# david-m-rosen/Optimization

Hardware: AMD Instinct MI355X
Metric: TNT Steihaug-CG HVP+inner-product throughput (higher is better)
Workload: dtype f64

## Files before the change

optimization_amd/csrc/context.hip:

```cpp
#include "mi_internal.h"
#include <chrono>
#include <cstring>
#include <strings.h>
#include <unistd.h>

#include <dlfcn.h>

namespace mi {

static thread_local char g_err[1024] = "";

void set_error(const char *fmt, ...) {
  va_list ap;
  va_start(ap, fmt);
  vsnprintf(g_err, sizeof(g_err), fmt, ap);
  va_end(ap);
}

int hip_fail(hipError_t e, const char *what, const char *file, int line) {
  set_error("HIP error %d (%s) in %s at %s:%d", (int)e, hipGetErrorString(e), what, file, line);
  (void)hipGetLastError();
  if (e == hipErrorNoDevice || e == hipErrorInvalidDevice) return MI_ERR_NO_DEVICE;
  if (e == hipErrorOutOfMemory) return MI_ERR_OOM;
  return MI_ERR_HIP;
// ... 171 lines not shown
using namespace mi;

namespace {
struct OptionDesc {
  const char *name;
  int (*set)(mi_ctx *, long);
  bool integer = false;
};
#define OPT_BOOL(FN, FIELD) \
  int FN(mi_ctx *c, long v) { c->FIELD = v != 0; return MI_OK; }
OPT_BOOL(opt_force_slot_path, force_slot_path)
OPT_BOOL(opt_force_lockstep, force_lockstep)
OPT_BOOL(opt_no_dirgram, no_dirgram)
OPT_BOOL(opt_dirgram_direct, dirgram_direct)
OPT_BOOL(opt_force_uniform_grid, cfg.force_uniform_grid)
OPT_BOOL(opt_no_fold, cfg.no_fold)
OPT_BOOL(opt_halo_push_late, cfg.halo_push_late)
OPT_BOOL(opt_no_packed, cfg.no_packed)
OPT_BOOL(opt_no_window, cfg.no_window)
OPT_BOOL(opt_no_win_bounds, cfg.no_win_bounds)
OPT_BOOL(opt_no_far_computed, cfg.no_far_computed)
OPT_BOOL(opt_words16, cfg.words16)
OPT_BOOL(opt_no_spmm_stream, cfg.no_spmm_stream)
OPT_BOOL(opt_no_spmm_win, cfg.no_spmm_win)
OPT_BOOL(opt_no_spmm_sweep, cfg.no_spmm_sweep)
OPT_BOOL(opt_no_zero_copy, cfg.no_zero_copy)
OPT_BOOL(opt_no_polled_sync, cfg.no_polled_sync)
OPT_BOOL(opt_no_update_mfma, cfg.no_update_mfma)
OPT_BOOL(opt_halo_rprime, cfg.halo_rprime)
OPT_BOOL(opt_no_gram_half, cfg.no_gram_half)
OPT_BOOL(opt_so3_no_quat, cfg.so3_no_quat)
OPT_BOOL(opt_so3_no_rquat, cfg.so3_no_rquat)
OPT_BOOL(opt_early_s, cfg.early_s)
OPT_BOOL(opt_no_update_pair, cfg.no_update_pair)
OPT_BOOL(opt_two_kernel_step, cfg.two_kernel_step)
OPT_BOOL(opt_warn_generic, warn_generic)
#undef OPT_BOOL
int opt_max_grid(mi_ctx *c, long v) {
  c->max_grid = (int)std::min<long>(kMaxGrid, std::max<long>(1, v));
  return MI_OK;
}
int opt_wide_quad(mi_ctx *c, long v) {
  c->cfg.wide_quad = v < 0 ? -1 : v != 0;
  return MI_OK;
}
int opt_wide_window(mi_ctx *c, long v) {
  c->cfg.wide_window = v < 0 ? -1 : v != 0;
  return MI_OK;
}
int opt_so3_sort_nbr(mi_ctx *c, long v) {
  c->cfg.so3_sort_nbr = (int)v;
  return MI_OK;
}
int opt_sweep_zsegs(mi_ctx *c, long v) {
  c->cfg.sweep_zsegs = (int)std::max<long>(0, std::min<long>(v, 1024));
  return MI_OK;
}
int opt_reanchor(mi_ctx *c, long v) {
  c->cfg.reanchor = (int)std::max<long>(0, std::min<long>(v, 1 << 20));
  return MI_OK;
}
int opt_ipc_timeout_ms(mi_ctx *c, long v) {
  c->cfg.ipc_timeout_ms = std::max<long>(0, v);
  return MI_OK;
}
const OptionDesc kOptions[] = {
    {"FORCE_SLOT_PATH", opt_force_slot_path}, {"FORCE_LOCKSTEP", opt_force_lockstep},
    {"NO_DIRGRAM", opt_no_dirgram}, {"DIRGRAM_DIRECT", opt_dirgram_direct}, {"MAX_GRID", opt_max_grid, true},
    {"FORCE_UNIFORM_GRID", opt_force_uniform_grid}, {"IPC_TIMEOUT_MS", opt_ipc_timeout_ms, true},
    {"NO_FOLD", opt_no_fold}, {"HALO_PUSH_LATE", opt_halo_push_late}, {"NO_PACKED", opt_no_packed},
    {"NO_WINDOW", opt_no_window}, {"NO_WIN_BOUNDS", opt_no_win_bounds}, {"NO_FAR_COMPUTED", opt_no_far_computed},
    {"WORDS16", opt_words16}, {"NO_SPMM_STREAM", opt_no_spmm_stream}, {"NO_SPMM_WIN", opt_no_spmm_win},
    {"NO_SPMM_SWEEP", opt_no_spmm_sweep}, {"SWEEP_ZSEGS", opt_sweep_zsegs, true},
    {"NO_ZERO_COPY", opt_no_zero_copy}, {"NO_POLLED_SYNC", opt_no_polled_sync}, {"WIDE_QUAD", opt_wide_quad, true}, {"WIDE_WINDOW", opt_wide_window, true},
    {"NO_UPDATE_MFMA", opt_no_update_mfma}, {"HALO_RPRIME", opt_halo_rprime}, {"NO_GRAM_HALF", opt_no_gram_half}, {"SO3_NO_QUAT", opt_so3_no_quat}, {"SO3_NO_RQUAT", opt_so3_no_rquat}, {"EARLY_S", opt_early_s}, {"NO_UPDATE_PAIR", opt_no_update_pair}, {"TWO_KERNEL_STEP", opt_two_kernel_step}, {"SO3_SORT_NBR", opt_so3_sort_nbr, true},
    {"WARN_GENERIC", opt_warn_generic}, {"REANCHOR", opt_reanchor, true},
};
bool option_value(const OptionDesc &o, const char *e, long *v) {
  char *end = nullptr;
  *v = strtol(e, &end, 0);
  if (end != e && *end == '\0') return true;
  if (o.integer) {
    fprintf(stderr, "[mi355opt] warning: MI355OPT_%s=\"%s\" is not an integer; ignored (the default stays)\n", o.name, e);
    return false;
  }
  *v = (!strcasecmp(e, "no") || !strcasecmp(e, "false") || !strcasecmp(e, "off")) ? 0 : 1;
  return true;
}
void config_from_env(mi_ctx *ctx) {
  for (const OptionDesc &o : kOptions) {
    char name[64];
    snprintf(name, sizeof(name), "MI355OPT_%s", o.name);
    long v = 0;
    if (const char *e = getenv(name))
      if (option_value(o, e, &v)) (void)o.set(ctx, v);
  }
  static bool warned = false;
  if (warned || !environ) return;
  warned = true;
  for (char **ep = environ; *ep; ++ep) {
    if (strncmp(*ep, "MI355OPT_", 9) != 0) continue;
    const char *nm = *ep + 9, *eq = strchr(nm, '=');
    const size_t len = eq ? (size_t)(eq - nm) : strlen(nm);
    bool known = false;
    for (const OptionDesc &o : kOptions) known |= strlen(o.name) == len && strncmp(o.name, nm, len) == 0;
    for (const char *h : {"LIB", "COMM", "BUILD_TAG", "EXTRA_CFLAGS", "NO_UNITY"})
      known |= strlen(h) == len && strncmp(h, nm, len) == 0;
    known |= len >= 6 && strncmp(nm, "BENCH_", 6) == 0;
// ... 297 lines not shown
```

optimization_amd/csrc/mi_internal.h:

```cpp
#pragma once

#include <hip/hip_runtime.h>

#include <cstdarg>
#include <cstdint>
#include <cstdio>
#include <cstring>
#include <map>
#include <string>
#include <set>
#include <vector>

#include "mi355opt.h"

namespace mi {

constexpr int kWave = 64;
constexpr int kBlock = 1024;
constexpr int kWaves = kBlock / kWave;
constexpr int kMaxP = 8;
constexpr int kMaxGrid = 512;
constexpr int kMaxRows = 1024;
constexpr int kMaxComps = 64;
constexpr int kNumXCD = 8;
// ... 41 lines not shown
};
static_assert(sizeof(CgState) <= 128, "the CG state is meant to fit one 128-byte line");
struct CgConst {
  double Delta, Delta_2, epsilon;
  unsigned long long max_iterations;
  unsigned long long rag0, rag_per;
};
enum CgMode { CG_RUN = 0, CG_KERNEL_PENDING = 1, CG_APPLY_SIGMA = 2, CG_DONE = 3 };

struct Config {
  bool force_uniform_grid = false;
  long ipc_timeout_ms = 0;
  bool no_fold = false;
  bool halo_push_late = false;
  bool no_packed = false;
  bool no_window = false;
  bool no_win_bounds = false;
  bool no_far_computed = false;
  bool words16 = false;
  bool no_spmm_stream = false;
  bool no_spmm_sweep = true;
  int sweep_zsegs = 0;
  bool no_spmm_win = false;
  bool no_zero_copy = false;
  int wide_quad = -1;
  int wide_window = -1;
  bool no_polled_sync = false;
  bool two_kernel_step = false;
  int reanchor = 25;
  bool no_update_pair = false;
  bool no_gram_half = false;
  bool no_update_mfma = false;
  bool halo_rprime = false;
  bool early_s = false;
  bool so3_no_rquat = false;
  bool so3_no_quat = false;
  int so3_sort_nbr = 0;
};

struct KTimer {
  bool enabled = false;
  std::vector<std::pair<hipEvent_t, hipEvent_t>> pending;
  size_t launches = 0;
  double total_ms = 0;
};

}

struct mi_ctx {
  int device = -1;
  hipStream_t stream = nullptr;
  char device_name[128] = {0};
  int num_cu = 256;
  bool uniform_grid = false;
  int max_grid = 512;
  std::multimap<size_t, void *> pool_free;
  std::map<void *, size_t> pool_all;
  size_t pool_bytes = 0;
  void *control_slab = nullptr;
  double *partials = nullptr;
  double *partials_b = nullptr;
  double *partials2 = nullptr;
  double *partials_user = nullptr;
  double *scalars = nullptr;
  double *host_scalars = nullptr;
  mi::CgState *cg = nullptr;
// ... 367 lines not shown
```

optimization_amd/csrc/stpcg.hip:

```cpp
#include "comm_ipc.h"
#include "mi_internal.h"
#include "stiefel_core.h"

#include <cmath>
#include <type_traits>

using namespace mi;

namespace {

enum { PRE_NONE = 0, PRE_DIAG = 1, PRE_BLOCK3 = 2, PRE_EXTERNAL = 3 };

__device__ __forceinline__ void publish(HostStatus *hs, unsigned long long launches, int done) {
  __hip_atomic_store(&hs->word, (uint64_t)(launches << 1) | (uint64_t)(done ? 1 : 0), __ATOMIC_RELAXED,
                     __HIP_MEMORY_SCOPE_SYSTEM);
}

#define CG_FIELDS(X)                                                                               \
  X(sk_M_pk) X(sk_M_2) X(pk_M_2) X(target_rk_norm) X(rv) X(alpha) X(beta)                          \
  X(kappa) X(sigma) X(skplus1_M_2) X(M_norm) X(k) X(launches) X(mode) X(exit_reason)
__device__ __forceinline__ CgState load_state(const CgState *__restrict__ src) {
  CgState s;
#define X(f) s.f = src->f;
  CG_FIELDS(X)
// ... 257 lines not shown
    s.mode = CG_DONE;
    s.exit_reason = MI_STPCG_EXIT_RESIDUAL;
    s.M_norm = sqrt(0.0);
  }
  store_state(st, s);
  publish(hs, 0, s.mode == CG_DONE);
}

struct DirGramArgs {
  const double *X, *Y, *S;
  double *gpartials;
  double *gdir;
  int ns;
};

#ifdef MI_FOLD_STAMPS
}
extern "C" __attribute__((visibility("default"))) int mi_debug_fold_stamp_buffer(void *dev_ptr) {
  return (int)hipMemcpyToSymbol(HIP_SYMBOL(mi::g_fold_stamps), &dev_ptr, sizeof(dev_ptr));
}
namespace {
#endif

template <int SP>
struct DirGramLds {
  static constexpr int value = (SymIdx<SP>::NS * kWaves > kWaves + 1) ? SymIdx<SP>::NS * kWaves : kWaves + 1;
};
template <>
struct DirGramLds<0> {
  static constexpr int value = kWaves + 1;
};
static_assert(kWaves + 1 >= kIpcVals, "LDS of the folded exchange");

#define CG_KERNEL_ATTR
#define CG_UPDATE_NAME k_cg_update
#define CG_PUPDATE_NAME k_cg_pupdate
#include "stpcg_kernels.inc"
#undef CG_KERNEL_ATTR
#undef CG_UPDATE_NAME
#undef CG_PUPDATE_NAME
#define CG_KERNEL_ATTR __attribute__((amdgpu_num_sgpr(80), amdgpu_waves_per_eu(8, 8)))
#define CG_UPDATE_NAME k_cg_update_s80
#define CG_PUPDATE_NAME k_cg_pupdate_s80
#include "stpcg_kernels.inc"
#undef CG_KERNEL_ATTR
#undef CG_UPDATE_NAME
#undef CG_PUPDATE_NAME

template <class F>
__device__ __forceinline__ void reduce_rows_1x512(const double *__restrict__ partials, int count, double &out, double *lds,
                                                  F &&after_issue) {
  const int lane = threadIdx.x & 63, w = threadIdx.x >> 6;
  double t[8];
#pragma unroll
  for (int j = 0; j < 8; ++j) t[j] = 0.0;
  if (w == 0) {
#pragma unroll
    for (int j = 0; j < 8; ++j) {
      const int r = lane + 64 * j;
      if (r < count) t[j] = partials[r];
    }
  }
  after_issue();
  if (w == 0) {
    double v = 0;
#pragma unroll
    for (int j = 0; j < 8; ++j) v += t[j];
    v = wave_reduce_sum(v);
    if (lane == 0) lds[0] = v;
  }
  __syncthreads();
  out = lds[0];
  __syncthreads();
}

__global__ __launch_bounds__(kBlock) __attribute__((amdgpu_waves_per_eu(8, 8))) void k_cg_pupdate_early(
    size_t n, CgConst cc, const CgState *__restrict__ st_in, CgState *__restrict__ st_out,
    const double *__restrict__ partials_b, int nparts_b, const double *__restrict__ v, double *__restrict__ p,
    double *__restrict__ s, HostStatus *hs, double *__restrict__ trace, size_t trace_cap, DirGramArgs dg) {
  __shared__ double lds[kWaves + 1];
// ... 224 lines not shown
__global__ __launch_bounds__(kBlock) void k_cg_dirgram2(size_t nrows, const CgState *__restrict__ st,
                                                        const double *__restrict__ va, const double *__restrict__ vb,
                                                        DirGramArgs dg) {
  static_assert(SP >= 1 && SP <= 4, "narrow rows");
  __shared__ double lds[SymIdx<SP>::NS * kWaves];
  if (st->mode != CG_RUN) return;
  double Sm[SP * SP], Ga[SP * SP], Gb[SP * SP];
#pragma unroll
  for (int i = 0; i < SP * SP; ++i) { Ga[i] = 0; Gb[i] = 0; Sm[i] = dg.S[i]; }
  const size_t stride = (size_t)gridDim.x * kBlock;
  for (size_t row = (size_t)blockIdx.x * kBlock + threadIdx.x; row < nrows; row += stride) {
    double x[SP], y[SP], a[SP], b[SP];
#pragma unroll
    for (int c = 0; c < SP; ++c) {
      x[c] = dg.X[row * SP + c]; y[c] = dg.Y[row * SP + c]; a[c] = va[row * SP + c]; b[c] = vb[row * SP + c];
    }
#pragma unroll
    for (int j = 0; j < SP; ++j) {
      double ta = 0, tb = 0;
#pragma unroll
      for (int i = 0; i < SP; ++i) { ta += a[i] * Sm[i * SP + j]; tb += b[i] * Sm[i * SP + j]; }
#pragma unroll
      for (int i = 0; i < SP; ++i) {
        Ga[i * SP + j] += y[i] * a[j] - x[i] * ta;
        Gb[i * SP + j] += y[i] * b[j] - x[i] * tb;
      }
    }
  }
  store_sym_partials<SP>(Ga, lds, dg.gpartials);
  __syncthreads();
  store_sym_partials<SP>(Gb, lds, dg.gpartials + (size_t)SymIdx<SP>::NS * kMaxRows);
}

template <int SP>
__global__ __launch_bounds__(StBlk<SP>::threads) void k_cg_init_dirgram(size_t nrows, const double *__restrict__ g,
                                                            double *__restrict__ r, double *__restrict__ p,
                                                            double *__restrict__ s, double *__restrict__ partials,
                                                            DirGramArgs dg) {
  constexpr int BLK = StBlk<SP>::threads, NW = StBlk<SP>::waves;
  constexpr bool WIDE = SP > 4;
  __shared__ double lds[SymIdx<SP>::NS * NW];
  __shared__ double SmL[WIDE ? SP * SP : 1];
  double Sm[WIDE ? 1 : SP * SP], G[SP * SP];
#pragma unroll
  for (int i = 0; i < SP * SP; ++i) G[i] = 0;
  if (WIDE) {
    if (threadIdx.x < SP * SP) SmL[threadIdx.x] = dg.S[threadIdx.x];
    __syncthreads();
  } else {
#pragma unroll
    for (int i = 0; i < SP * SP; ++i) Sm[WIDE ? 0 : i] = dg.S[i];
  }
  double acc[1] = {0};
  const size_t stride = (size_t)gridDim.x * BLK;
  for (size_t row = (size_t)blockIdx.x * BLK + threadIdx.x; row < nrows; row += stride) {
    double x[SP], y[SP], gv[SP], pv[SP];
#pragma unroll
    for (int c = 0; c < SP; ++c) { x[c] = dg.X[row * SP + c]; y[c] = dg.Y[row * SP + c]; gv[c] = g[row * SP + c]; }
#pragma unroll
    for (int c = 0; c < SP; ++c) {
      pv[c] = -gv[c];
      r[row * SP + c] = gv[c];
      s[row * SP + c] = 0 * gv[c];
      p[row * SP + c] = pv[c];
      acc[0] += gv[c] * gv[c];
    }
    if (WIDE) asm volatile("" ::: "memory");
#pragma unroll
    for (int b = 0; b < SP; ++b) {
      double t = 0;
#pragma unroll
      for (int a = 0; a < SP; ++a) t += pv[a] * (WIDE ? SmL[a * SP + b] : Sm[WIDE ? 0 : a * SP + b]);
#pragma unroll
      for (int a = 0; a < SP; ++a) G[a * SP + b] += y[a] * pv[b] - x[a] * t;
    }
  }
  store_sym_partials<SP>(G, lds, dg.gpartials);
  __syncthreads();
  block_partials_store_w<1, NW>(acc, lds, partials);
}

__global__ __launch_bounds__(kBlock) void k_cg_gdir_init(const double *__restrict__ partials, int count, int ns,
                                                         const double *__restrict__ slots, int from_slots,
                                                         double *__restrict__ gdir) {
  if (!from_slots) {
    gdir_from_rows(partials, count, ns, gdir);
    return;
  }
  if (threadIdx.x < ns) {
    const double v = slots[threadIdx.x];
    gdir[SLOT_GDIR_P + threadIdx.x] = v;
    gdir[threadIdx.x] = -v;
  }
}

__global__ __launch_bounds__(kBlock) void k_cg_gdir_anchor(const double *__restrict__ partials, int count, int ns,
// ... 179 lines not shown
  hipStream_t st = ctx->stream;
  const int grid = (pre == PRE_BLOCK3) ? grid_for(ctx, n / 3, 2) : grid_for(ctx, n, 4);
  {
    const size_t n2 = n >> 1, step = (size_t)grid * kBlock;
    cc.rag0 = (n2 / step) * step;
    cc.rag_per = (n2 - cc.rag0 + (size_t)grid - 1) / (size_t)grid;
  }
  const bool recur = dgp && pre == PRE_NONE && !ctx->dirgram_direct;
  const int gns = dgp ? dgp->p * (dgp->p + 1) / 2 : 0;
  const DirGramArgs dga = dgp ? DirGramArgs{dgp->X, dgp->Y, dgp->S, ctx->partials2,
                                            recur ? ctx->scalars + SLOT_GDIR : nullptr, gns}
                              : DirGramArgs{nullptr, nullptr, nullptr, nullptr, nullptr, 0};
  const int sp = (dgp && !recur) ? dgp->p : 0;
  const int kc = recur ? dir_comps(dgp->p) : 3;
  double *slots_g = ctx->scalars + SLOT_GRAM;
  double *slots_a = ctx->scalars + SLOT_CG, *slots_b = ctx->scalars + SLOT_CG + 4;
  CgState *st0 = ctx->cg, *st1 = ctx->cg1;
  const bool folded = sharded && recur && kc <= kIpcVals && comm_fold_enabled(ctx) && !ctx->force_slot_path;
  bool rprime = false;
  if (recur && !folded && dgp->halo_A) {
    const int st_rp = comm_rprime_prepare(ctx, dgp->halo_A, &rprime);
    if (st_rp != MI_OK) {
      mi_vec_destroy(r);
      mi_vec_destroy(p);
      mi_vec_destroy(Hp);
      if (v) mi_vec_destroy(v);
      return st_rp;
    }
  }
  const bool init_fused = recur && n == dgp->n * (size_t)dgp->p;
  const bool gdir_in_scalar_init = recur && !sharded && !rows;
  const bool twok = ctx->cfg.two_kernel_step && recur && dgp->twok && dgp->p == 3 && !sharded && !rows && !lockstep &&
                    init_fused && gdir_in_scalar_init;
  CgState *st_final = st0;
  double *tr = tcap ? ctx->trace_dev : nullptr;
  int ret = MI_OK;
  ctx->cg_live = st0;

#define CG_CHECK(expr)   \
  do {                   \
    int _s = (expr);     \
    if (_s != MI_OK) {   \
      ret = _s;          \
      goto cleanup;      \
    }                    \
  } while (0)
#define LAUNCH_PRE(KERNEL, ...)                                                                   \
  switch (pre) {                                                                                  \
    case PRE_NONE: hipLaunchKernelGGL((KERNEL<PRE_NONE>), dim3(grid), dim3(kBlock), 0, st, __VA_ARGS__); break;     \
    case PRE_DIAG: hipLaunchKernelGGL((KERNEL<PRE_DIAG>), dim3(grid), dim3(kBlock), 0, st, __VA_ARGS__); break;     \
    case PRE_BLOCK3: hipLaunchKernelGGL((KERNEL<PRE_BLOCK3>), dim3(grid), dim3(kBlock), 0, st, __VA_ARGS__); break; \
    default: hipLaunchKernelGGL((KERNEL<PRE_EXTERNAL>), dim3(grid), dim3(kBlock), 0, st, __VA_ARGS__); break;       \
  }
#define LAUNCH_UPDATE(FS)                                                                              \
  switch (pre) {                                                                                       \
    case PRE_NONE: hipLaunchKernelGGL((k_cg_update<PRE_NONE, FS>), dim3(grid), dim3(kBlock), 0, st, UPD_ARGS, NoFold{}); break;     \
    case PRE_DIAG: hipLaunchKernelGGL((k_cg_update<PRE_DIAG, FS>), dim3(grid), dim3(kBlock), 0, st, UPD_ARGS, NoFold{}); break;     \
    case PRE_BLOCK3: hipLaunchKernelGGL((k_cg_update<PRE_BLOCK3, FS>), dim3(grid), dim3(kBlock), 0, st, UPD_ARGS, NoFold{}); break; \
    default: hipLaunchKernelGGL((k_cg_update<PRE_EXTERNAL, FS>), dim3(grid), dim3(kBlock), 0, st, UPD_ARGS, NoFold{}); break;       \
  }

  if (init_fused) {
    KScope ks(ctx, MI_K_CG_INIT);
    const size_t nrows = dgp->n;
#define INIT_DG(SPV)                                                                                       \
  hipLaunchKernelGGL(k_cg_init_dirgram<SPV>, dim3(grid), dim3(StBlk<SPV>::threads), 0, st, nrows, (const double *)g->d, \
                     r->d, p->d, s_out->d, ctx->partials_b, dga)
    switch (dgp->p) {
      case 1: INIT_DG(1); break;
      case 2: INIT_DG(2); break;
      case 3: INIT_DG(3); break;
      case 4: INIT_DG(4); break;
      case 5: INIT_DG(5); break;
      case 6: INIT_DG(6); break;
      case 7: INIT_DG(7); break;
      default: INIT_DG(8); break;
    }
#undef INIT_DG
  } else {
    KScope ks(ctx, MI_K_CG_INIT);
    LAUNCH_PRE(k_cg_init, n, (const double *)g->d, pred, r->d, vd, p->d, s_out->d, ctx->partials_b);
  }
  if (pre == PRE_EXTERNAL) {
    if (P->apply_project) CG_CHECK(P->apply_project(P, r, v, prm->constraint_At));
    else CG_CHECK(P->apply(P, r, v));
    hipLaunchKernelGGL(k_cg_dot_rv<true>, dim3(grid), dim3(kBlock), 0, st, n, (const CgState *)st0,
                       (const double *)r->d, (const double *)v->d, p->d, ctx->partials_b);
  }
  if (dgp) {
    const size_t nrows = dgp->n;
    if (!init_fused) {
      switch (dgp->p) {
        case 1: hipLaunchKernelGGL(k_cg_dirgram<1>, dim3(grid), dim3(kBlock), 0, st, nrows, (const double *)p->d, dga); break;
        case 2: hipLaunchKernelGGL(k_cg_dirgram<2>, dim3(grid), dim3(kBlock), 0, st, nrows, (const double *)p->d, dga); break;
        case 3: hipLaunchKernelGGL(k_cg_dirgram<3>, dim3(grid), dim3(kBlock), 0, st, nrows, (const double *)p->d, dga); break;
        case 4: hipLaunchKernelGGL(k_cg_dirgram<4>, dim3(grid), dim3(kBlock), 0, st, nrows, (const double *)p->d, dga); break;
        case 5: hipLaunchKernelGGL(k_cg_dirgram<5>, dim3(grid), dim3(StBlk<5>::threads), 0, st, nrows, (const double *)p->d, dga); break;
        case 6: hipLaunchKernelGGL(k_cg_dirgram<6>, dim3(grid), dim3(StBlk<6>::threads), 0, st, nrows, (const double *)p->d, dga); break;
        case 7: hipLaunchKernelGGL(k_cg_dirgram<7>, dim3(grid), dim3(StBlk<7>::threads), 0, st, nrows, (const double *)p->d, dga); break;
        default: hipLaunchKernelGGL(k_cg_dirgram<8>, dim3(grid), dim3(StBlk<8>::threads), 0, st, nrows, (const double *)p->d, dga); break;
// ... 81 lines not shown
                             ctx->status_dev, tr, tcap, dga);
        }
        st_final = nxt;
        continue;
      }
      if (dgp) {
        CG_CHECK(H->apply_dir(H, p, Hp, recur ? -1 : grid, &nparts));
      } else if (H->apply_dots) {
        CG_CHECK(H->apply_dots(H, p, Hp, &nparts));
      } else {
        CG_CHECK(H->apply(H, p, Hp));
        CG_CHECK(launch_dot3_partials(ctx, n, p->d, Hp->d, &nparts));
      }
      ++hvp;
#define UPD_ARGS                                                                                      \
  n, cc, (const CgState *)st0, st1, (const double *)ctx->partials, nparts,                              \
      (const double *)(recur ? slots_g : slots_a), (const double *)p->d, (const double *)Hp->d, pred,  \
      s_out->d, r->d, vd, ctx->partials_b, dga
      if (recur) {
#define UPD_RECUR(KN, FS, FT, FV)                                                                                  \
  switch (kc) {                                                                                                    \
    case 4: hipLaunchKernelGGL((KN<PRE_NONE, FS, 4, FT>), dim3(grid), dim3(kBlock), 0, st, UPD_ARGS, FV); break;   \
    case 6: hipLaunchKernelGGL((KN<PRE_NONE, FS, 6, FT>), dim3(grid), dim3(kBlock), 0, st, UPD_ARGS, FV); break;   \
    case 9: hipLaunchKernelGGL((KN<PRE_NONE, FS, 9, FT>), dim3(grid), dim3(kBlock), 0, st, UPD_ARGS, FV); break;   \
    default: hipLaunchKernelGGL((k_cg_update_s80<PRE_NONE, FS, 16, FT>), dim3(grid), dim3(kBlock), 0, st, UPD_ARGS, FV); break; \
  }
#define UPD_WIDE(FS)                                                                                                        \
  switch (kc) {                                                                                                             \
    case 18: hipLaunchKernelGGL((k_cg_update<PRE_NONE, FS, 18, NoFold>), dim3(grid), dim3(kBlock), 0, st, UPD_ARGS, NoFold{}); break; \
    case 24: hipLaunchKernelGGL((k_cg_update<PRE_NONE, FS, 24, NoFold>), dim3(grid), dim3(kBlock), 0, st, UPD_ARGS, NoFold{}); break; \
    case 31: hipLaunchKernelGGL((k_cg_update<PRE_NONE, FS, 31, NoFold>), dim3(grid), dim3(kBlock), 0, st, UPD_ARGS, NoFold{}); break; \
    default: hipLaunchKernelGGL((k_cg_update<PRE_NONE, FS, 39, NoFold>), dim3(grid), dim3(kBlock), 0, st, UPD_ARGS, NoFold{}); break; \
  }
        if (kc > 16) {
          if (sharded) CG_CHECK(reduce_rows_allreduce(ctx, ctx->partials, nparts, kc, slots_g));
          else if (rows) CG_CHECK(comm_allreduce_rows(ctx, ctx->partials, kc));
          KScope ks(ctx, MI_K_CG_UPDATE);
          if (sharded) { UPD_WIDE(true); } else { UPD_WIDE(false); }
        } else if (sharded && folded) {
          const FoldArgs fold_a = comm_fold_next(ctx);
          KScope ks(ctx, MI_K_CG_UPDATE);
          UPD_RECUR(k_cg_update_s80, false, FoldArgs, fold_a);
        } else if (sharded) {
          CG_CHECK(reduce_rows_allreduce(ctx, ctx->partials, nparts, kc, slots_g));
          KScope ks(ctx, MI_K_CG_UPDATE);
          UPD_RECUR(k_cg_update_s80, true, NoFold, NoFold{});
        } else {
          if (rows) CG_CHECK(comm_allreduce_rows(ctx, ctx->partials, kc));
          KScope ks(ctx, MI_K_CG_UPDATE);
          UPD_RECUR(k_cg_update, false, NoFold, NoFold{});
        }
#undef UPD_RECUR
#undef UPD_WIDE
      } else if (sharded) {
        CG_CHECK(reduce_rows_allreduce(ctx, ctx->partials, nparts, 3, slots_a));
        KScope ks(ctx, MI_K_CG_UPDATE);
        LAUNCH_UPDATE(true);
      } else {
        if (rows) CG_CHECK(comm_allreduce_rows(ctx, ctx->partials, 3));
        KScope ks(ctx, MI_K_CG_UPDATE);
        LAUNCH_UPDATE(false);
      }
#undef UPD_ARGS
      if (pre == PRE_EXTERNAL) {
        if (P->apply_project) CG_CHECK(P->apply_project(P, r, v, prm->constraint_At));
        else CG_CHECK(P->apply(P, r, v));
        hipLaunchKernelGGL(k_cg_dot_rv<false>, dim3(grid), dim3(kBlock), 0, st, n, (const CgState *)st1,
                           (const double *)r->d, (const double *)v->d, p->d, ctx->partials_b);
      }
#define PUPD_ARGS                                                                                          \
  n, cc, (const CgState *)st1, st0, (const double *)ctx->partials_b, grid, (const double *)slots_b,        \
      (const double *)vd, p->d, s_out->d, ctx->status_dev, tr, tcap, dga
#define PUPD(KN, FS, SPV) \
  hipLaunchKernelGGL((KN<FS, SPV>), dim3(grid), dim3(kBlock), 0, st, PUPD_ARGS, NoFold{})
#define LAUNCH_PUPD(KN0, KN1, FS)               \
  switch (sp) {                                 \
    case 0: PUPD(KN0, FS, 0); break;            \
    case 1: PUPD(KN1, FS, 1); break;            \
    case 2: PUPD(k_cg_pupdate, FS, 2); break;   \
    case 3: PUPD(k_cg_pupdate, FS, 3); break;   \
    default: PUPD(k_cg_pupdate, FS, 4); break;  \
  }
      if (sharded && folded) {
        const FoldArgs fold_b = comm_fold_next(ctx);
        FoldPush fp{fold_b, HaloPush{}};
        const bool push = dgp && dgp->halo_A && k + 1 < prm->max_iterations &&
                          comm_halo_fold_next(ctx, dgp->halo_A, dgp->p, p->d, &fp.h);
        KScope ks(ctx, MI_K_CG_PUPDATE);
        if (push)
          hipLaunchKernelGGL((k_cg_pupdate_s80<false, 0, FoldPush>), dim3(grid), dim3(kBlock), 0, st, PUPD_ARGS, fp);
        else
          hipLaunchKernelGGL((k_cg_pupdate_s80<false, 0, FoldArgs>), dim3(grid), dim3(kBlock), 0, st, PUPD_ARGS, fold_b);
      } else if (sharded) {
        CG_CHECK(reduce_rows_allreduce(ctx, ctx->partials_b, grid, 1, slots_b));
        if (rprime) CG_CHECK(comm_rprime_exchange(ctx, dgp->halo_A, dgp->p, r->d, nullptr, 0));
        KScope ks(ctx, MI_K_CG_PUPDATE);
        LAUNCH_PUPD(k_cg_pupdate_s80, k_cg_pupdate_s80, true);
      } else {
        if (rows && rprime) CG_CHECK(comm_rprime_exchange(ctx, dgp->halo_A, dgp->p, r->d, ctx->partials_b, 1));
        else if (rows) CG_CHECK(comm_allreduce_rows(ctx, ctx->partials_b, 1));
        KScope ks(ctx, MI_K_CG_PUPDATE);
        const bool early = sp == 0 && !rows && ctx->cfg.early_s && grid <= 512 && cc.rag0 <= 2ull * (size_t)grid * kBlock &&
                           (n >> 1) < ((size_t)1 << 31);
        if (early)
          hipLaunchKernelGGL(k_cg_pupdate_early, dim3(grid), dim3(kBlock), 0, st, n, cc, (const CgState *)st1, st0,
                             (const double *)ctx->partials_b, grid, (const double *)vd, p->d, s_out->d, ctx->status_dev, tr,
                             tcap, dga);
        else
          LAUNCH_PUPD(k_cg_pupdate, k_cg_pupdate_s80, false);
      }
      if (rprime && (sharded || rows)) {
        const double *hr = nullptr;
        double *hp = nullptr;
        size_t cnt = 0;
        comm_rprime_buffers(ctx, dgp->halo_A, dgp->p, &hr, &hp, &cnt);
        if (cnt) {
          const int hg = (int)std::max<size_t>(1, std::min<size_t>((cnt + 255) / 256, 512));
          hipLaunchKernelGGL(k_halo_dir, dim3(hg), dim3(256), 0, st, (const CgState *)st0, hr, hp, cnt);
        }
        comm_rprime_mark(ctx, dgp->halo_A, dgp->p, p->d);
      }
#undef LAUNCH_PUPD
#undef PUPD
#undef PUPD_ARGS
    }
    result->hvp_calls = hvp;
    comm_halo_fold_drop(ctx);
  }

  if (prm->defer_result && !(trace && trace->cap)) {
    hipError_t e = hipSuccess;
    *precon_fail_host(ctx) = 0.0;
    ctx->cg_deferred_seq = result_to_host(ctx, st_final, P);
    if (!ctx->cg_deferred_seq) {
      if (!ctx->cg_deferred_ev) e = hipEventCreateWithFlags(&ctx->cg_deferred_ev, hipEventDisableTiming);
      if (e == hipSuccess) e = hipMemcpyAsync(ctx->cg_host, st_final, sizeof(CgState), hipMemcpyDeviceToHost, st);
      if (e == hipSuccess && P && P->fail_word)
// ... 68 lines not shown
```

optimization_amd/csrc/stpcg_kernels.inc:

```

template <int PRE, bool FROM_SLOTS, int KC = 3, class FOLD = NoFold>
__global__ __launch_bounds__(kBlock) CG_KERNEL_ATTR void CG_UPDATE_NAME(size_t n, CgConst cc, const CgState *__restrict__ st_in,
                                                      CgState *__restrict__ st_out,
                                                      const double *__restrict__ partials_a, int nparts_a,
                                                      const double *__restrict__ slots,
                                                      const double *__restrict__ p,
                                                      const double *__restrict__ Hp,
                                                      const double *__restrict__ pre,
                                                      double *__restrict__ s, double *__restrict__ r,
                                                      double *__restrict__ v,
                                                      double *__restrict__ partials_b, DirGramArgs dg,
                                                      FOLD fold) {
  __shared__ double lds[3 * (kWaves + 1)];
  static_assert(KC >= 3 && KC <= 3 * (kWaves + 1), "3 curvature dots + at most 36 Gram components (p <= 8)");
  CgState cs = load_state(st_in);
  if (cs.mode == CG_DONE) {
    if (blockIdx.x == 0 && threadIdx.x == 0) store_state(st_out, cs);
    return;
  }
  FOLD_STAMP(0);
  const size_t n2 = n >> 1, stride = (size_t)gridDim.x * kBlock;
  const size_t i0 = (size_t)blockIdx.x * kBlock + threadIdx.x;
  auto next_of = [&](size_t i_) -> size_t { return i_ + stride; };
  const size_t ifirst = i0;
  double2 hv0 = make_double2(0, 0), rv0 = hv0;
  constexpr bool kFolded = !std::is_same<FOLD, NoFold>::value;
  auto prefetch_now = [&] {
    if (PRE != PRE_BLOCK3 && ifirst < n2) {
      hv0 = reinterpret_cast<const double2 *>(Hp)[ifirst];
      rv0 = reinterpret_cast<double2 *>(r)[ifirst];
    }
  };
  auto prefetch = [&] {
    if (kFolded && threadIdx.x < 64) return;
    prefetch_now();
  };
  double d[KC];
  if (FROM_SLOTS) {
    prefetch_now();
#pragma unroll
    for (int i = 0; i < KC; ++i) d[i] = slots[i];
  } else {
    reduce_rows<KC>(partials_a, nparts_a, d, lds, prefetch);
    fold_maybe<KC>(d, fold, lds);
    if (kFolded && threadIdx.x < 64) prefetch_now();
    if (!kFolded) FOLD_STAMP(1);
  }
  step_a(cs, cc, d[0], d[1], d[2]);
  if (!kFolded) FOLD_STAMP(5);
  if (blockIdx.x == 0 && threadIdx.x == 0) {
    store_state(st_out, cs);
    if (KC > 3 && cs.mode == CG_RUN) {
#pragma unroll
      for (int i = 0; i < KC - 3; ++i)
        if (i < dg.ns) dg.gdir[i] = dg.gdir[i] + cs.alpha * d[3 + i];
    }
  }

  const int mode = cs.mode;
  double acc[1] = {0};
  if (mode == CG_APPLY_SIGMA) {
    const double sigma = cs.sigma;
    for (size_t i = i0; i < n2; i += stride) {
      const double2 pv = reinterpret_cast<const double2 *>(p)[i];
      double2 sv = reinterpret_cast<double2 *>(s)[i];
      sv.x += sigma * pv.x; sv.y += sigma * pv.y;
      reinterpret_cast<double2 *>(s)[i] = sv;
    }
    if ((n & 1) && blockIdx.x == 0 && threadIdx.x == 0) s[n - 1] += sigma * p[n - 1];
    return;
  }
  if (mode == CG_KERNEL_PENDING) {
    for (size_t i = i0; i < n2; i += stride) {
      const double2 pv = reinterpret_cast<const double2 *>(p)[i];
      const double2 rv = reinterpret_cast<const double2 *>(r)[i];
      acc[0] += pv.x * rv.x; acc[0] += pv.y * rv.y;
    }
    if ((n & 1) && blockIdx.x == 0 && threadIdx.x == 0) acc[0] += p[n - 1] * r[n - 1];
  } else {
    const double alpha = cs.alpha;
    if (PRE == PRE_BLOCK3) {
      const size_t nb = n / 3;
      for (size_t b = i0; b < nb; b += stride) {
        double rr[3];
#pragma unroll
        for (int c = 0; c < 3; ++c) {
          const size_t i = 3 * b + c;
          rr[c] = r[i] + alpha * Hp[i];
          r[i] = rr[c];
        }
        const double *M = pre + 9 * b;
#pragma unroll
        for (int c = 0; c < 3; ++c) {
          const double vv = M[3 * c] * rr[0] + M[3 * c + 1] * rr[1] + M[3 * c + 2] * rr[2];
          v[3 * b + c] = vv;
          acc[0] += rr[c] * vv;
        }
      }
    } else {
      double2 hv = hv0, rv = rv0;
      for (size_t i = ifirst; i < n2;) {
        const size_t inext = next_of(i);
        double2 hn = hv, rn = rv;
        if (inext < n2) {
          hn = reinterpret_cast<const double2 *>(Hp)[inext];
          rn = reinterpret_cast<double2 *>(r)[inext];
        }
        rv.x += alpha * hv.x; rv.y += alpha * hv.y;
        reinterpret_cast<double2 *>(r)[i] = rv;
        if (PRE != PRE_EXTERNAL) {
          double2 vv = rv;
          if (PRE == PRE_DIAG) {
            const double2 dd = reinterpret_cast<const double2 *>(pre)[i];
            vv.x = dd.x * rv.x; vv.y = dd.y * rv.y;
            reinterpret_cast<double2 *>(v)[i] = vv;
          }
          acc[0] += rv.x * vv.x; acc[0] += rv.y * vv.y;
        }
        i = inext; hv = hn; rv = rn;
      }
      if ((n & 1) && blockIdx.x == 0 && threadIdx.x == 0) {
        const size_t i = n - 1;
        const double rv = r[i] + alpha * Hp[i];
        r[i] = rv;
        if (PRE != PRE_EXTERNAL) {
          double vv = rv;
          if (PRE == PRE_DIAG) { vv = pre[i] * rv; v[i] = vv; }
          acc[0] += rv * vv;
        }
      }
    }
    if (PRE == PRE_EXTERNAL) return;
  }
  block_partials_store<1>(acc, lds, partials_b);
  FOLD_STAMP(6);
}

template <bool FROM_SLOTS, int SP, class FOLD = NoFold>
__global__ __launch_bounds__(kBlock) CG_KERNEL_ATTR void CG_PUPDATE_NAME(size_t n, CgConst cc, const CgState *__restrict__ st_in,
                                                       CgState *__restrict__ st_out,
                                                       const double *__restrict__ partials_b, int nparts_b,
                                                       const double *__restrict__ slots,
                                                       const double *__restrict__ v,
                                                       double *__restrict__ p, double *__restrict__ s,
                                                       HostStatus *hs, double *__restrict__ trace,
                                                       size_t trace_cap, DirGramArgs dg, FOLD fold) {
  __shared__ double lds[DirGramLds<SP>::value];
  CgState cs = load_state(st_in);
  const bool leader = blockIdx.x == 0 && threadIdx.x == 0;
  if (cs.mode == CG_DONE) {
    if (leader) store_state(st_out, cs);
    return;
  }
  const int mode_in = cs.mode;
  const size_t n2 = n >> 1, stride = (size_t)gridDim.x * kBlock;
  const size_t i0 = (size_t)blockIdx.x * kBlock + threadIdx.x;
  const size_t tail0 = cc.rag0, per = cc.rag_per;
  const size_t irem = (threadIdx.x < per) ? tail0 + (size_t)blockIdx.x * per + threadIdx.x : n2;
  auto next_of = [&](size_t i_) -> size_t {
    const size_t j_ = i_ + stride;
    return j_ < tail0 ? j_ : ((i_ < tail0 && irem < n2) ? irem : n2);
  };
  const size_t ifirst = i0 < tail0 ? i0 : (irem < n2 ? irem : n2);
  double2 vv0 = make_double2(0, 0), pv0 = vv0, sv0 = vv0;
  constexpr int SPN = SP > 0 ? SP : 1;
  double rv0[SPN], rp0[SPN], rs0[SPN], rx0[SPN], ry0[SPN];
#pragma unroll
  for (int c = 0; c < SPN; ++c) { rv0[c] = 0; rp0[c] = 0; rs0[c] = 0; rx0[c] = 0; ry0[c] = 0; }
  auto prefetch_now = [&] {
    if (SP > 0) {
      if (mode_in == CG_RUN && i0 < n / SPN) {
#pragma unroll
        for (int c = 0; c < SPN; ++c) {
          rv0[c] = v[i0 * SPN + c];
          rp0[c] = p[i0 * SPN + c];
          rs0[c] = s[i0 * SPN + c];
          rx0[c] = dg.X[i0 * SPN + c];
          ry0[c] = dg.Y[i0 * SPN + c];
        }
      }
    } else if (ifirst < n2) {
      const size_t q0 = halo_phys(fold, ifirst);
      vv0 = reinterpret_cast<const double2 *>(v)[q0];
      pv0 = reinterpret_cast<double2 *>(p)[q0];
      sv0 = reinterpret_cast<double2 *>(s)[q0];
    }
  };
  double red[1] = {0};
  if (mode_in != CG_APPLY_SIGMA && !FROM_SLOTS) {
    reduce_rows<1>(partials_b, nparts_b, red, lds, prefetch_now);
    fold_maybe<1>(red, fold, lds);
  } else {
    prefetch_now();
    if (mode_in != CG_APPLY_SIGMA) red[0] = slots[0];
  }
  step_b(cs, cc, red[0]);
  cs.launches = cs.launches + 1;
  if (leader) {
    store_state(st_out, cs);
    if (mode_in == CG_RUN && trace && cs.k - 1 < trace_cap) {
      const size_t k = (size_t)(cs.k - 1);
      trace[k] = cs.alpha;
      trace[trace_cap + k] = cs.beta;
      trace[2 * trace_cap + k] = cs.kappa;
      trace[3 * trace_cap + k] = cs.rv;
    }
    publish(hs, cs.launches, cs.mode == CG_DONE);
    if (SP == 0 && dg.gdir && mode_in == CG_RUN && cs.mode == CG_RUN) {
      for (int i = 0; i < dg.ns; ++i) dg.gdir[SLOT_GDIR_P + i] = -dg.gdir[i] + cs.beta * dg.gdir[SLOT_GDIR_P + i];
    }
  }
  if (mode_in == CG_KERNEL_PENDING) {
    const double sigma = cs.sigma;
    for (size_t i = i0; i < n2; i += stride) {
      const double2 pv = reinterpret_cast<const double2 *>(p)[i];
      double2 sv = reinterpret_cast<double2 *>(s)[i];
      sv.x += sigma * pv.x; sv.y += sigma * pv.y;
      reinterpret_cast<double2 *>(s)[i] = sv;
    }
    if ((n & 1) && leader) s[n - 1] += sigma * p[n - 1];
  } else if (mode_in == CG_RUN) {
    const double alpha = cs.alpha, beta = cs.beta;
    const bool dir = cs.mode == CG_RUN;
    if (SP > 0) {
      const size_t nrows = n / SPN;
      double Sm[SPN * SPN], G[SPN * SPN];
#pragma unroll
      for (int i = 0; i < SPN * SPN; ++i) { Sm[i] = dg.S[i]; G[i] = 0; }
      double rv[SPN], rp[SPN], rs[SPN], x[SPN], y[SPN];
#pragma unroll
      for (int c = 0; c < SPN; ++c) { rv[c] = rv0[c]; rp[c] = rp0[c]; rs[c] = rs0[c]; x[c] = rx0[c]; y[c] = ry0[c]; }
      for (size_t row = i0; row < nrows;) {
        const size_t rnext = row + stride;
        double vn[SPN], pn[SPN], sn[SPN], xn[SPN], yn[SPN];
#pragma unroll
        for (int c = 0; c < SPN; ++c) { vn[c] = rv[c]; pn[c] = rp[c]; sn[c] = rs[c]; xn[c] = x[c]; yn[c] = y[c]; }
        if (rnext < nrows) {
#pragma unroll
          for (int c = 0; c < SPN; ++c) {
            vn[c] = v[rnext * SPN + c];
            pn[c] = p[rnext * SPN + c];
            sn[c] = s[rnext * SPN + c];
            xn[c] = dg.X[rnext * SPN + c];
            yn[c] = dg.Y[rnext * SPN + c];
          }
        }
#pragma unroll
        for (int c = 0; c < SPN; ++c) {
          rs[c] = rs[c] + alpha * rp[c];
          s[row * SPN + c] = rs[c];
        }
        if (dir) {
#pragma unroll
          for (int c = 0; c < SPN; ++c) {
            rp[c] = -rv[c] + beta * rp[c];
            p[row * SPN + c] = rp[c];
          }
#pragma unroll
          for (int b = 0; b < SPN; ++b) {
            double t = 0;
#pragma unroll
            for (int a = 0; a < SPN; ++a) t += rp[a] * Sm[a * SPN + b];
#pragma unroll
            for (int a = 0; a < SPN; ++a) G[a * SPN + b] += y[a] * rp[b] - x[a] * t;
          }
        }
        row = rnext;
#pragma unroll
        for (int c = 0; c < SPN; ++c) { rv[c] = vn[c]; rp[c] = pn[c]; rs[c] = sn[c]; x[c] = xn[c]; y[c] = yn[c]; }
      }
      if (dir) store_sym_partials<SPN>(G, lds, dg.gpartials);
      return;
    }
    double2 vv = vv0, pv = pv0, sv = sv0;
    bool pushed = false;
    for (size_t L = ifirst; L < n2;) {
      const size_t Lnext = next_of(L), q = halo_phys(fold, L);
      double2 vn = vv, pn = pv, sn = sv;
      if (Lnext < n2) {
        const size_t qn = halo_phys(fold, Lnext);
        vn = reinterpret_cast<const double2 *>(v)[qn];
        pn = reinterpret_cast<double2 *>(p)[qn];
        sn = reinterpret_cast<double2 *>(s)[qn];
      }
      sv.x = sv.x + alpha * pv.x; sv.y = sv.y + alpha * pv.y;
      reinterpret_cast<double2 *>(s)[q] = sv;
      if (dir) {
        pv.x = -vv.x + beta * pv.x; pv.y = -vv.y + beta * pv.y;
        reinterpret_cast<double2 *>(p)[q] = pv;
        pushed |= halo_push_store(fold, q, pv);
        if (L == ifirst) halo_push_first_step_done(fold);
      }
      L = Lnext; vv = vn; pv = pn; sv = sn;
    }
    if ((n & 1) && leader) {
      s[n - 1] = s[n - 1] + alpha * p[n - 1];
      if (dir) p[n - 1] = -v[n - 1] + beta * p[n - 1];
    }
    if (dir) halo_push_finish(fold, pushed);
  }
}
```

Baseline: 5686.

## Skip r/s initialization writes and read g directly in first CG iteration

The fused CG init kernel no longer writes r=g and s=0. Specialized first-iteration update and p-update kernels (G0 variants) instead read g directly and synthesize p=-g and s=0 in registers. This removes one full-vector write pass at setup and the matching reads in iteration zero, at the cost of more kernel instantiations and extra dispatch branches. The new path is on by default and can be disabled with the LEGACY_SETUP option.

```diff
diff --git a/optimization_amd/csrc/context.hip b/optimization_amd/csrc/context.hip
--- a/optimization_amd/csrc/context.hip
+++ b/optimization_amd/csrc/context.hip
@@ -227,6 +227,7 @@
 OPT_BOOL(opt_so3_no_quat, cfg.so3_no_quat)
 OPT_BOOL(opt_so3_no_rquat, cfg.so3_no_rquat)
 OPT_BOOL(opt_early_s, cfg.early_s)
+OPT_BOOL(opt_legacy_setup, cfg.legacy_setup)
 OPT_BOOL(opt_no_update_pair, cfg.no_update_pair)
 OPT_BOOL(opt_two_kernel_step, cfg.two_kernel_step)
 OPT_BOOL(opt_warn_generic, warn_generic)
@@ -268,7 +269,7 @@
     {"WORDS16", opt_words16}, {"NO_SPMM_STREAM", opt_no_spmm_stream}, {"NO_SPMM_WIN", opt_no_spmm_win},
     {"NO_SPMM_SWEEP", opt_no_spmm_sweep}, {"SWEEP_ZSEGS", opt_sweep_zsegs, true},
     {"NO_ZERO_COPY", opt_no_zero_copy}, {"NO_POLLED_SYNC", opt_no_polled_sync}, {"WIDE_QUAD", opt_wide_quad, true}, {"WIDE_WINDOW", opt_wide_window, true},
-    {"NO_UPDATE_MFMA", opt_no_update_mfma}, {"HALO_RPRIME", opt_halo_rprime}, {"NO_GRAM_HALF", opt_no_gram_half}, {"SO3_NO_QUAT", opt_so3_no_quat}, {"SO3_NO_RQUAT", opt_so3_no_rquat}, {"EARLY_S", opt_early_s}, {"NO_UPDATE_PAIR", opt_no_update_pair}, {"TWO_KERNEL_STEP", opt_two_kernel_step}, {"SO3_SORT_NBR", opt_so3_sort_nbr, true},
+    {"NO_UPDATE_MFMA", opt_no_update_mfma}, {"HALO_RPRIME", opt_halo_rprime}, {"NO_GRAM_HALF", opt_no_gram_half}, {"SO3_NO_QUAT", opt_so3_no_quat}, {"SO3_NO_RQUAT", opt_so3_no_rquat}, {"EARLY_S", opt_early_s}, {"LEGACY_SETUP", opt_legacy_setup}, {"NO_UPDATE_PAIR", opt_no_update_pair}, {"TWO_KERNEL_STEP", opt_two_kernel_step}, {"SO3_SORT_NBR", opt_so3_sort_nbr, true},
     {"WARN_GENERIC", opt_warn_generic}, {"REANCHOR", opt_reanchor, true},
 };
 bool option_value(const OptionDesc &o, const char *e, long *v) {
diff --git a/optimization_amd/csrc/mi_internal.h b/optimization_amd/csrc/mi_internal.h
--- a/optimization_amd/csrc/mi_internal.h
+++ b/optimization_amd/csrc/mi_internal.h
@@ -97,6 +97,7 @@
   bool no_gram_half = false;
   bool no_update_mfma = false;
   bool halo_rprime = false;
+  bool legacy_setup = false;
   bool early_s = false;
   bool so3_no_rquat = false;
   bool so3_no_quat = false;
diff --git a/optimization_amd/csrc/stpcg.hip b/optimization_amd/csrc/stpcg.hip
--- a/optimization_amd/csrc/stpcg.hip
+++ b/optimization_amd/csrc/stpcg.hip
@@ -313,6 +313,7 @@
 };
 static_assert(kWaves + 1 >= kIpcVals, "LDS of the folded exchange");
 
+#define CG_G0 0
 #define CG_KERNEL_ATTR
 #define CG_UPDATE_NAME k_cg_update
 #define CG_PUPDATE_NAME k_cg_pupdate
@@ -327,6 +328,23 @@
 #undef CG_KERNEL_ATTR
 #undef CG_UPDATE_NAME
 #undef CG_PUPDATE_NAME
+#undef CG_G0
+#define CG_G0 1
+#define CG_KERNEL_ATTR
+#define CG_UPDATE_NAME k_cg_update_g0
+#define CG_PUPDATE_NAME k_cg_pupdate_g0
+#include "stpcg_kernels.inc"
+#undef CG_KERNEL_ATTR
+#undef CG_UPDATE_NAME
+#undef CG_PUPDATE_NAME
+#define CG_KERNEL_ATTR __attribute__((amdgpu_num_sgpr(80), amdgpu_waves_per_eu(8, 8)))
+#define CG_UPDATE_NAME k_cg_update_g0_s80
+#define CG_PUPDATE_NAME k_cg_pupdate_g0_s80
+#include "stpcg_kernels.inc"
+#undef CG_KERNEL_ATTR
+#undef CG_UPDATE_NAME
+#undef CG_PUPDATE_NAME
+#undef CG_G0
 
 template <class F>
 __device__ __forceinline__ void reduce_rows_1x512(const double *__restrict__ partials, int count, double &out, double *lds,
@@ -617,7 +635,7 @@
   store_sym_partials<SP>(Gb, lds, dg.gpartials + (size_t)SymIdx<SP>::NS * kMaxRows);
 }
 
-template <int SP>
+template <int SP, bool SETUP = false>
 __global__ __launch_bounds__(StBlk<SP>::threads) void k_cg_init_dirgram(size_t nrows, const double *__restrict__ g,
                                                             double *__restrict__ r, double *__restrict__ p,
                                                             double *__restrict__ s, double *__restrict__ partials,
@@ -645,8 +663,10 @@
 #pragma unroll
     for (int c = 0; c < SP; ++c) {
       pv[c] = -gv[c];
-      r[row * SP + c] = gv[c];
-      s[row * SP + c] = 0 * gv[c];
+      if (!SETUP) {
+        r[row * SP + c] = gv[c];
+        s[row * SP + c] = 0 * gv[c];
+      }
       p[row * SP + c] = pv[c];
       acc[0] += gv[c] * gv[c];
     }
@@ -892,6 +912,7 @@
   const bool gdir_in_scalar_init = recur && !sharded && !rows;
   const bool twok = ctx->cfg.two_kernel_step && recur && dgp->twok && dgp->p == 3 && !sharded && !rows && !lockstep &&
                     init_fused && gdir_in_scalar_init;
+  const bool setup = init_fused && gdir_in_scalar_init && !twok && !ctx->cfg.legacy_setup && prm->max_iterations > 0;
   CgState *st_final = st0;
   double *tr = tcap ? ctx->trace_dev : nullptr;
   int ret = MI_OK;
@@ -923,9 +944,13 @@
   if (init_fused) {
     KScope ks(ctx, MI_K_CG_INIT);
     const size_t nrows = dgp->n;
-#define INIT_DG(SPV)                                                                                       \
-  hipLaunchKernelGGL(k_cg_init_dirgram<SPV>, dim3(grid), dim3(StBlk<SPV>::threads), 0, st, nrows, (const double *)g->d, \
-                     r->d, p->d, s_out->d, ctx->partials_b, dga)
+#define INIT_DG(SPV)                                                                                                  \
+  if (setup)                                                                                                          \
+    hipLaunchKernelGGL((k_cg_init_dirgram<SPV, true>), dim3(grid), dim3(StBlk<SPV>::threads), 0, st, nrows,           \
+                       (const double *)g->d, r->d, p->d, s_out->d, ctx->partials_b, dga);                             \
+  else                                                                                                                \
+    hipLaunchKernelGGL((k_cg_init_dirgram<SPV, false>), dim3(grid), dim3(StBlk<SPV>::threads), 0, st, nrows,          \
+                       (const double *)g->d, r->d, p->d, s_out->d, ctx->partials_b, dga)
     switch (dgp->p) {
       case 1: INIT_DG(1); break;
       case 2: INIT_DG(2); break;
@@ -1073,11 +1098,10 @@
     case 31: hipLaunchKernelGGL((k_cg_update<PRE_NONE, FS, 31, NoFold>), dim3(grid), dim3(kBlock), 0, st, UPD_ARGS, NoFold{}); break; \
     default: hipLaunchKernelGGL((k_cg_update<PRE_NONE, FS, 39, NoFold>), dim3(grid), dim3(kBlock), 0, st, UPD_ARGS, NoFold{}); break; \
   }
-        if (kc > 16) {
-          if (sharded) CG_CHECK(reduce_rows_allreduce(ctx, ctx->partials, nparts, kc, slots_g));
-          else if (rows) CG_CHECK(comm_allreduce_rows(ctx, ctx->partials, kc));
+        if (kc > 16 && sharded) {
+          CG_CHECK(reduce_rows_allreduce(ctx, ctx->partials, nparts, kc, slots_g));
           KScope ks(ctx, MI_K_CG_UPDATE);
-          if (sharded) { UPD_WIDE(true); } else { UPD_WIDE(false); }
+          UPD_WIDE(true);
         } else if (sharded && folded) {
           const FoldArgs fold_a = comm_fold_next(ctx);
           KScope ks(ctx, MI_K_CG_UPDATE);
@@ -1086,6 +1110,28 @@
           CG_CHECK(reduce_rows_allreduce(ctx, ctx->partials, nparts, kc, slots_g));
           KScope ks(ctx, MI_K_CG_UPDATE);
           UPD_RECUR(k_cg_update_s80, true, NoFold, NoFold{});
+        } else if (setup && k == 0) {
+#define UPD_ARGS_G0                                                                                                \
+  n, cc, (const CgState *)st0, st1, (const double *)ctx->partials, nparts, (const double *)slots_g,                 \
+      (const double *)p->d, (const double *)Hp->d, (const double *)g->d, s_out->d, r->d, vd, ctx->partials_b, dga, NoFold{}
+#define UPD_G0(KN, KCV) hipLaunchKernelGGL((KN<PRE_NONE, false, KCV, NoFold>), dim3(grid), dim3(kBlock), 0, st, UPD_ARGS_G0)
+          KScope ks(ctx, MI_K_CG_UPDATE);
+          switch (kc) {
+            case 4: UPD_G0(k_cg_update_g0_s80, 4); break;
+            case 6: UPD_G0(k_cg_update_g0_s80, 6); break;
+            case 9: UPD_G0(k_cg_update_g0_s80, 9); break;
+            case 16: UPD_G0(k_cg_update_g0_s80, 16); break;
+            case 18: UPD_G0(k_cg_update_g0, 18); break;
+            case 24: UPD_G0(k_cg_update_g0, 24); break;
+            case 31: UPD_G0(k_cg_update_g0, 31); break;
+            default: UPD_G0(k_cg_update_g0, 39); break;
+          }
+#undef UPD_G0
+#undef UPD_ARGS_G0
+        } else if (kc > 16) {
+          if (rows) CG_CHECK(comm_allreduce_rows(ctx, ctx->partials, kc));
+          KScope ks(ctx, MI_K_CG_UPDATE);
+          UPD_WIDE(false);
         } else {
           if (rows) CG_CHECK(comm_allreduce_rows(ctx, ctx->partials, kc));
           KScope ks(ctx, MI_K_CG_UPDATE);
@@ -1143,7 +1189,11 @@
         KScope ks(ctx, MI_K_CG_PUPDATE);
         const bool early = sp == 0 && !rows && ctx->cfg.early_s && grid <= 512 && cc.rag0 <= 2ull * (size_t)grid * kBlock &&
                            (n >> 1) < ((size_t)1 << 31);
-        if (early)
+        if (setup && k == 0)
+          hipLaunchKernelGGL((k_cg_pupdate_g0_s80<false, 0, NoFold>), dim3(grid), dim3(kBlock), 0, st, n, cc,
+                             (const CgState *)st1, st0, (const double *)ctx->partials_b, grid, (const double *)g->d,
+                             (const double *)vd, p->d, s_out->d, ctx->status_dev, tr, tcap, dga, NoFold{});
+        else if (early)
           hipLaunchKernelGGL(k_cg_pupdate_early, dim3(grid), dim3(kBlock), 0, st, n, cc, (const CgState *)st1, st0,
                              (const double *)ctx->partials_b, grid, (const double *)vd, p->d, s_out->d, ctx->status_dev, tr,
                              tcap, dga);
diff --git a/optimization_amd/csrc/stpcg_kernels.inc b/optimization_amd/csrc/stpcg_kernels.inc
--- a/optimization_amd/csrc/stpcg_kernels.inc
+++ b/optimization_amd/csrc/stpcg_kernels.inc
@@ -13,9 +13,20 @@
                                                       FOLD fold) {
   __shared__ double lds[3 * (kWaves + 1)];
   static_assert(KC >= 3 && KC <= 3 * (kWaves + 1), "3 curvature dots + at most 36 Gram components (p <= 8)");
+#if CG_G0
+  static_assert(PRE == PRE_NONE && !FROM_SLOTS && std::is_same<FOLD, NoFold>::value, "G0: one rank, no preconditioner");
+  const double *__restrict__ g0 = pre;
+#endif
   CgState cs = load_state(st_in);
   if (cs.mode == CG_DONE) {
     if (blockIdx.x == 0 && threadIdx.x == 0) store_state(st_out, cs);
+#if CG_G0
+    for (size_t i = (size_t)blockIdx.x * kBlock + threadIdx.x; i < (n >> 1); i += (size_t)gridDim.x * kBlock) {
+      const double2 gv = reinterpret_cast<const double2 *>(g0)[i];
+      reinterpret_cast<double2 *>(s)[i] = make_double2(0 * gv.x, 0 * gv.y);
+    }
+    if ((n & 1) && blockIdx.x == 0 && threadIdx.x == 0) s[n - 1] = 0 * g0[n - 1];
+#endif
     return;
   }
   FOLD_STAMP(0);
@@ -28,7 +39,11 @@
   auto prefetch_now = [&] {
     if (PRE != PRE_BLOCK3 && ifirst < n2) {
       hv0 = reinterpret_cast<const double2 *>(Hp)[ifirst];
+#if CG_G0
+      rv0 = reinterpret_cast<const double2 *>(g0)[ifirst];
+#else
       rv0 = reinterpret_cast<double2 *>(r)[ifirst];
+#endif
     }
   };
   auto prefetch = [&] {
@@ -63,20 +78,37 @@
     const double sigma = cs.sigma;
     for (size_t i = i0; i < n2; i += stride) {
       const double2 pv = reinterpret_cast<const double2 *>(p)[i];
+#if CG_G0
+      const double2 gv = reinterpret_cast<const double2 *>(g0)[i];
+      double2 sv = make_double2(0 * gv.x, 0 * gv.y);
+#else
       double2 sv = reinterpret_cast<double2 *>(s)[i];
+#endif
       sv.x += sigma * pv.x; sv.y += sigma * pv.y;
       reinterpret_cast<double2 *>(s)[i] = sv;
     }
+#if CG_G0
+    if ((n & 1) && blockIdx.x == 0 && threadIdx.x == 0) s[n - 1] = 0 * g0[n - 1] + sigma * p[n - 1];
+#else
     if ((n & 1) && blockIdx.x == 0 && threadIdx.x == 0) s[n - 1] += sigma * p[n - 1];
+#endif
     return;
   }
   if (mode == CG_KERNEL_PENDING) {
     for (size_t i = i0; i < n2; i += stride) {
       const double2 pv = reinterpret_cast<const double2 *>(p)[i];
+#if CG_G0
+      const double2 rv = reinterpret_cast<const double2 *>(g0)[i];
+#else
       const double2 rv = reinterpret_cast<const double2 *>(r)[i];
+#endif
       acc[0] += pv.x * rv.x; acc[0] += pv.y * rv.y;
     }
+#if CG_G0
+    if ((n & 1) && blockIdx.x == 0 && threadIdx.x == 0) acc[0] += p[n - 1] * g0[n - 1];
+#else
     if ((n & 1) && blockIdx.x == 0 && threadIdx.x == 0) acc[0] += p[n - 1] * r[n - 1];
+#endif
   } else {
     const double alpha = cs.alpha;
     if (PRE == PRE_BLOCK3) {
@@ -104,7 +136,11 @@
         double2 hn = hv, rn = rv;
         if (inext < n2) {
           hn = reinterpret_cast<const double2 *>(Hp)[inext];
+#if CG_G0
+          rn = reinterpret_cast<const double2 *>(g0)[inext];
+#else
           rn = reinterpret_cast<double2 *>(r)[inext];
+#endif
         }
         rv.x += alpha * hv.x; rv.y += alpha * hv.y;
         reinterpret_cast<double2 *>(r)[i] = rv;
@@ -121,7 +157,11 @@
       }
       if ((n & 1) && blockIdx.x == 0 && threadIdx.x == 0) {
         const size_t i = n - 1;
+#if CG_G0
+        const double rv = g0[i] + alpha * Hp[i];
+#else
         const double rv = r[i] + alpha * Hp[i];
+#endif
         r[i] = rv;
         if (PRE != PRE_EXTERNAL) {
           double vv = rv;
@@ -146,6 +186,10 @@
                                                        HostStatus *hs, double *__restrict__ trace,
                                                        size_t trace_cap, DirGramArgs dg, FOLD fold) {
   __shared__ double lds[DirGramLds<SP>::value];
+#if CG_G0
+  static_assert(SP == 0 && !FROM_SLOTS && std::is_same<FOLD, NoFold>::value, "G0: one rank, recurrence form");
+  const double *__restrict__ g0 = slots;
+#endif
   CgState cs = load_state(st_in);
   const bool leader = blockIdx.x == 0 && threadIdx.x == 0;
   if (cs.mode == CG_DONE) {
@@ -182,8 +226,14 @@
     } else if (ifirst < n2) {
       const size_t q0 = halo_phys(fold, ifirst);
       vv0 = reinterpret_cast<const double2 *>(v)[q0];
+#if CG_G0
+      const double2 gv = reinterpret_cast<const double2 *>(g0)[q0];
+      pv0 = make_double2(-gv.x, -gv.y);
+      sv0 = make_double2(0 * gv.x, 0 * gv.y);
+#else
       pv0 = reinterpret_cast<double2 *>(p)[q0];
       sv0 = reinterpret_cast<double2 *>(s)[q0];
+#endif
     }
   };
   double red[1] = {0};
@@ -213,12 +263,25 @@
   if (mode_in == CG_KERNEL_PENDING) {
     const double sigma = cs.sigma;
     for (size_t i = i0; i < n2; i += stride) {
+#if CG_G0
+      const double2 gv = reinterpret_cast<const double2 *>(g0)[i];
+      const double2 pv = make_double2(-gv.x, -gv.y);
+      double2 sv = make_double2(0 * gv.x, 0 * gv.y);
+#else
       const double2 pv = reinterpret_cast<const double2 *>(p)[i];
       double2 sv = reinterpret_cast<double2 *>(s)[i];
+#endif
       sv.x += sigma * pv.x; sv.y += sigma * pv.y;
       reinterpret_cast<double2 *>(s)[i] = sv;
     }
+#if CG_G0
+    if ((n & 1) && leader) {
+      const double gl = g0[n - 1], pl = -gl, sl = 0 * gl;
+      s[n - 1] = sl + sigma * pl;
+    }
+#else
     if ((n & 1) && leader) s[n - 1] += sigma * p[n - 1];
+#endif
   } else if (mode_in == CG_RUN) {
     const double alpha = cs.alpha, beta = cs.beta;
     const bool dir = cs.mode == CG_RUN;
@@ -280,8 +343,14 @@
       if (Lnext < n2) {
         const size_t qn = halo_phys(fold, Lnext);
         vn = reinterpret_cast<const double2 *>(v)[qn];
+#if CG_G0
+        const double2 gv = reinterpret_cast<const double2 *>(g0)[qn];
+        pn = make_double2(-gv.x, -gv.y);
+        sn = make_double2(0 * gv.x, 0 * gv.y);
+#else
         pn = reinterpret_cast<double2 *>(p)[qn];
         sn = reinterpret_cast<double2 *>(s)[qn];
+#endif
       }
       sv.x = sv.x + alpha * pv.x; sv.y = sv.y + alpha * pv.y;
       reinterpret_cast<double2 *>(s)[q] = sv;
@@ -294,8 +363,14 @@
       L = Lnext; vv = vn; pv = pn; sv = sn;
     }
     if ((n & 1) && leader) {
+#if CG_G0
+      const double gl = g0[n - 1], pl = -gl, sl = 0 * gl;
+      s[n - 1] = sl + alpha * pl;
+      if (dir) p[n - 1] = -v[n - 1] + beta * pl;
+#else
       s[n - 1] = s[n - 1] + alpha * p[n - 1];
       if (dir) p[n - 1] = -v[n - 1] + beta * p[n - 1];
+#endif
     }
     if (dir) halo_push_finish(fold, pushed);
   }
```

After: 5707 (median of 6 runs). Within noise of the previous version (+0.4%).
